# revvu/online_convex_optimization

Measured on AMD Instinct MI355X. Metric: FTRL timesteps/sec (whole node) at d=64, T=1e4; max |regret-ref| error, higher is better.
Workload: dtype f64; 1 GPU; configs[2]: batched FTRL d=64 T=1e4 (1e5-trial job as resident batches of B per GPU); B_per_gpu=32768, T=10000, d=64, coords_per_lane=8, lanes_mode=best, sums=butterfly, comparator=closed form T/2-||theta_T|| (certified per sequence), parallelism=dp1, z_bytes_per_gpu=167772160000

## Files before the change

### include/ocx_testing.h

```cpp
#ifndef OCX_TESTING_H_
#define OCX_TESTING_H_

#include <stdint.h>

#include "ocx.h"

#ifdef __cplusplus
extern "C" {
#endif

int ocx_test_gT_regrets_unclean(uint64_t base_seed, int64_t T, int64_t run0, int64_t R,
                                int64_t d, double eta0, double* regrets, int lanes_per_seq,
                                int device, int64_t unclean_every);

int ocx_test_alg_pipe_chunked(const ocx_layout* L, const double* z_tiled, const double* y_tiled,
                              double eta0, int64_t chunk_steps, double* regret, int* bad,
                              void* stream);

int ocx_test_alg_range(const ocx_layout* L, const double* z_tiled, const double* y_tiled,
                       double eta0, int onepass, int64_t g0, int64_t gn, double* regret,
                       double* gmax, void* stream);

int ocx_test_simulate_alg_etas(const ocx_layout* L, const double* z_tiled, const double* y_tiled,
                               const double* etas, int64_t M, double* regret, double* cum_loss,
                               double* comp_loss, int32_t* closed_out, int flags, int group,
                               void* stream);

int ocx_test_simulate_smart_thresholds(const ocx_layout* L, const double* z_tiled,
                                       const double* y_tiled, const double* thresh, int64_t M,
                                       double eta0, double* regret, int64_t* switch_step,
                                       int flags, unsigned long long* stats, int group,
                                       void* stream);

int64_t ocx_test_trailing_batches(void);

#ifdef __cplusplus
}
#endif
#endif
```

### online_convex_optimization_amd/_lib.py

```python
from __future__ import annotations

import ctypes
import os
import threading

_HERE = os.path.dirname(os.path.abspath(__file__))
LIB_PATH = os.environ.get("OCX_LIB", os.path.join(_HERE, "libocx.so"))

c_dp = ctypes.POINTER(ctypes.c_double)
c_i64p = ctypes.POINTER(ctypes.c_int64)
c_i64 = ctypes.c_int64
c_u64 = ctypes.c_uint64
c_int = ctypes.c_int
c_double = ctypes.c_double
c_vp = ctypes.c_void_p
c_fp = ctypes.POINTER(ctypes.c_float)


class OCXError(RuntimeError):
    """A libocx call failed (bad argument, HIP error, unsupported shape)."""


class Layout(ctypes.Structure):
    _fields_ = [("B", c_i64), ("T", c_i64), ("d", c_i64), ("P", ctypes.c_int32),
# ... 16 lines not shown
    "ocx_simulate_smart_batch": (c_int, [c_dp, c_dp, c_i64, c_i64, c_i64, c_dp, c_double, c_dp,
                                         c_i64p, c_int, c_int]),
    "ocx_ftl_exact_batch": (c_int, [c_dp, c_dp, c_i64, c_i64, c_i64, c_int, c_dp, c_dp, c_dp,
                                    ctypes.POINTER(ctypes.c_int32), c_int, c_int]),
    "ocx_dev_ftl_exact": (c_int, [ctypes.POINTER(Layout), c_vp, c_vp, c_int, c_vp, c_vp, c_vp, c_vp,
                                  c_vp]),
    "ocx_ftl_prefix_actions_batch": (c_int, [c_dp, c_dp, c_i64, c_i64, c_i64, c_int, c_dp,
                                             ctypes.POINTER(ctypes.c_int32), c_int, c_int]),
    "ocx_dev_ftl_prefix_actions": (c_int, [ctypes.POINTER(Layout), c_vp, c_vp, c_int, c_vp, c_vp,
                                           c_vp]),
    "ocx_ftrl_vs_exact_batch": (c_int, [c_dp, c_dp, c_i64, c_i64, c_i64, c_double, c_dp, c_dp,
                                        c_dp, c_dp, c_dp, ctypes.POINTER(ctypes.c_int32), c_int,
                                        c_int]),
    "ocx_ftrl_vs_exact_batch_ex": (c_int, [c_dp, c_dp, c_i64, c_i64, c_i64, c_double, c_dp, c_dp,
                                           c_dp, c_dp, c_dp, ctypes.POINTER(ctypes.c_int32),
                                           c_int, c_int, c_int]),
    "ocx_dev_ftrl_vs_exact": (c_int, [ctypes.POINTER(Layout), c_vp, c_vp, c_double, c_vp, c_vp,
                                      c_vp, c_vp, c_vp, c_vp, c_vp]),
    "ocx_replay_batch": (c_int, [c_dp, c_dp, c_dp, c_i64, c_i64, c_i64, c_dp, c_dp, c_int]),
    "ocx_gT_regrets": (c_int, [c_u64, c_i64, c_i64, c_i64, c_i64, c_double, c_dp, c_int, c_int]),
    "ocx_gT_regrets_dev": (c_int, [c_u64, c_i64, c_i64, c_i64, c_i64, c_double, c_vp, c_int,
                                   c_int]),
    "ocx_gT_max": (c_int, [c_u64, c_i64, c_i64, c_i64, c_i64, c_double, c_int, c_int, c_dp]),
    "ocx_dev_pack": (c_int, [ctypes.POINTER(Layout), c_vp, c_vp, c_vp, c_vp, c_vp]),
    "ocx_dev_gen_gT": (c_int, [ctypes.POINTER(Layout), c_u64, c_i64, c_vp, c_vp, c_vp]),
    "ocx_dev_gen_family": (c_int, [ctypes.POINTER(Layout), c_int, c_vp, c_vp, c_double, c_i64,
                                   c_vp, c_vp, c_vp]),
    "ocx_dev_simulate_alg": (c_int, [ctypes.POINTER(Layout), c_vp, c_vp, c_int, c_double, c_vp,
                                     c_vp, c_vp, c_vp, c_vp, c_vp]),
    "ocx_dev_simulate_smart": (c_int, [ctypes.POINTER(Layout), c_vp, c_vp, c_vp, c_double, c_vp,
                                       c_vp, c_vp]),
    "ocx_dev_simulate_smart_ex": (c_int, [ctypes.POINTER(Layout), c_vp, c_vp, c_vp, c_double,
                                          c_vp, c_vp, c_int, c_vp, c_vp]),
    "ocx_dev_replay": (c_int, [ctypes.POINTER(Layout), ctypes.POINTER(Layout), c_vp, c_vp, c_vp,
                               c_vp, c_vp, c_vp]),
    "ocx_dev_max_regret": (c_int, [c_vp, c_i64, c_vp, c_vp]),
    "ocx_dev_gen_simulate": (c_int, [ctypes.POINTER(Layout), c_u64, c_i64, c_i64, c_vp, c_vp,
                                     c_double, c_vp, c_vp, ctypes.c_uint32, c_i64, c_vp]),
    "ocx_dev_simulate_alg_ex": (c_int, [ctypes.POINTER(Layout), c_vp, c_vp, c_int, c_double, c_vp,
                                        c_vp, c_vp, c_vp, c_vp, c_int, c_vp, c_vp]),
    "ocx_curve_workspace_bytes": (c_i64, [ctypes.POINTER(Layout), c_i64]),
    "ocx_dev_simulate_alg_curve": (c_int, [ctypes.POINTER(Layout), c_vp, c_vp, c_int, c_double,
                                           c_vp, c_i64, c_vp, c_vp, c_vp, c_vp, c_int, c_vp,
                                           ctypes.c_size_t, c_vp]),
    "ocx_simulate_alg_curve_batch": (c_int, [c_dp, c_dp, c_i64, c_i64, c_i64, c_int, c_double,
                                             c_i64p, c_i64, c_dp, c_dp, c_dp,
                                             ctypes.POINTER(ctypes.c_int32), c_int, c_int]),
    "ocx_etas_group": (c_int, [ctypes.POINTER(Layout), c_i64]),
    "ocx_dev_simulate_alg_etas": (c_int, [ctypes.POINTER(Layout), c_vp, c_vp, c_dp, c_i64, c_vp,
                                          c_vp, c_vp, c_vp, c_int, c_vp]),
    "ocx_simulate_alg_etas_batch": (c_int, [c_dp, c_dp, c_i64, c_i64, c_i64, c_dp, c_i64, c_dp,
                                            c_dp, c_dp, ctypes.POINTER(ctypes.c_int32), c_int,
                                            c_int]),
    "ocx_smart_thresholds_group": (c_int, [ctypes.POINTER(Layout), c_i64]),
    "ocx_dev_simulate_smart_thresholds": (c_int, [ctypes.POINTER(Layout), c_vp, c_vp, c_vp, c_i64,
                                                  c_double, c_vp, c_vp, c_int, c_vp, c_vp]),
    "ocx_simulate_smart_thresholds_batch": (c_int, [c_dp, c_dp, c_i64, c_i64, c_i64, c_dp, c_i64,
                                                    c_double, c_dp, c_i64p, c_int, c_int]),
    "ocx_dev_ftrl_vs_exact_ex": (c_int,[ctypes.POINTER(Layout), c_vp, c_vp, c_double, c_vp, c_vp,
                                         c_vp, c_vp, c_vp, c_vp, c_int, c_int, c_vp]),
    "ocx_gT_sweep": (c_int, [c_i64p, c_int, c_i64, c_u64, c_i64, c_double, c_int, c_dp, c_dp]),
    "ocx_gT_sweep_devices": (c_int, [c_i64p, c_int, c_i64, c_u64, c_i64, c_double,
                                     ctypes.POINTER(c_int), c_int, c_int, c_dp, c_dp]),
    "ocx_comparator_loss_blas_batch": (c_int, [c_dp, c_dp, c_dp, c_i64, c_i64, c_i64, c_dp, c_int]),
    "ocx_twin32_batch": (c_int, [c_fp, c_fp, c_i64, c_i64, c_i64, c_int, c_double, c_dp, c_fp,
                                 c_dp, c_fp, c_i64p, c_int]),
    "ocx_dev_twin32": (c_int, [ctypes.POINTER(Layout), c_vp, c_vp, c_int, c_double, c_vp, c_vp,
                               c_vp, c_vp, c_vp, c_vp]),
    "ocx_twin32_gT_regrets": (c_int, [c_u64, c_i64, c_i64, c_i64, c_i64, c_double, c_fp, c_int]),
    "ocx_exact_ball_solve": (c_int, [c_dp, c_dp, c_i64, c_i64, c_i64, c_int, c_int, c_dp, c_dp,
                                     c_dp, c_dp, ctypes.POINTER(ctypes.c_int32), c_int]),
    "ocx_dev_exact_ball_solve": (c_int, [c_vp, c_vp, c_i64, c_i64, c_i64, c_int, c_int, c_vp, c_vp,
                                         c_vp, c_vp, c_vp, c_vp]),
    "ocx_dev_exact_ball_solve_tiled": (c_int, [ctypes.POINTER(Layout), c_vp, c_vp, c_int, c_int,
                                               c_vp, c_vp, c_vp, c_vp, c_vp, c_vp]),
}
TEST_SIGNATURES = {
    "ocx_test_gT_regrets_unclean": (c_int, [c_u64, c_i64, c_i64, c_i64, c_i64, c_double, c_dp,
                                            c_int, c_int, c_i64]),
    "ocx_test_alg_pipe_chunked": (c_int, [ctypes.POINTER(Layout), c_vp, c_vp, c_double, c_i64,
                                          c_vp, c_vp, c_vp]),
    "ocx_test_alg_range": (c_int, [ctypes.POINTER(Layout), c_vp, c_vp, c_double, c_int, c_i64,
                                   c_i64, c_vp, c_vp, c_vp]),
    "ocx_test_simulate_alg_etas": (c_int, [ctypes.POINTER(Layout), c_vp, c_vp, c_dp, c_i64, c_vp,
                                           c_vp, c_vp, c_vp, c_int, c_int, c_vp]),
    "ocx_test_simulate_smart_thresholds": (c_int, [ctypes.POINTER(Layout), c_vp, c_vp, c_vp, c_i64,
                                                   c_double, c_vp, c_vp, c_int, c_vp, c_int,
                                                   c_vp]),
    "ocx_test_trailing_batches": (c_i64, []),
}
OCX_VERSION = 400
OCX_ALG_CLIPPED_ROWS = 1
OCX_EXACT_BALL_MAX_D = 256
OCX_ALG_CLOSED_COMPARATOR = 2
OCX_ALG_TREE_SUMS = 4
OCX_SMART_CLOSED_PREFIX = 8
OCX_GENSIM_SEQUENTIAL = 1
OCX_GENSIM_TWO_PASS = 2

_lib = None
_lock = threading.Lock()


def _share_torch_hip_runtime() -> None:
    if os.environ.get("OCX_NO_TORCH"):
        return
    try:
        import torch
    except ImportError:
        pass


def load():
    global _lib
    if _lib is not None:
        return _lib
    with _lock:
        if _lib is None:
            _share_torch_hip_runtime()
            if not os.path.exists(LIB_PATH):
                raise OCXError(f"libocx.so not found at {LIB_PATH}: the HIP extension is not "
                               "built (python -m online_convex_optimization_amd._build)")
            lib = ctypes.CDLL(LIB_PATH)
            for name, (res, args) in {**SIGNATURES, **TEST_SIGNATURES}.items():
                fn = getattr(lib, name)
                fn.restype = res
                fn.argtypes = args
            if lib.ocx_version() != OCX_VERSION:
                raise OCXError(f"{LIB_PATH} implements ABI version {lib.ocx_version()}, this "
                               f"binding expects {OCX_VERSION}: rebuild the library")
            _lib = lib
    return _lib


def last_error() -> str:
    buf = ctypes.create_string_buffer(4096)
    load().ocx_last_error(buf, len(buf))
    return buf.value.decode(errors="replace")


def check(rc: int, what: str = "") -> None:
    if rc != 0:
        kind = {-1: "invalid argument", -2: "HIP error", -3: "unsupported"}.get(rc, str(rc))
        msg = f"{what}: {kind}: {last_error()}"
        if rc == -1:
            raise ValueError(msg)
        raise OCXError(msg)


def call(name: str, *args) -> None:
    check(getattr(load(), name)(*args), name)


def device_count() -> int:
    n = c_int(0)
    call("ocx_device_count", ctypes.byref(n))
    return int(n.value)


def release_buffers(device: int = 0) -> None:
    call("ocx_release_buffers", int(device))


def layout(B: int, T: int, d: int, lanes_per_seq: int = 0) -> Layout:
    L = Layout()
    call("ocx_layout_init", int(B), int(T), int(d), int(lanes_per_seq), ctypes.byref(L))
# ... 8 lines not shown
```

### online_convex_optimization_amd/csrc/ocx_alg_pipe.h

```cpp
#pragma once
#include <cstdlib>
#include <type_traits>
#include <utility>

#include "ocx_alg_step.h"
#include "ocx_sim_kernels.h"

#ifndef OCX_PIPE_IT32_MAXC
#define OCX_PIPE_IT32_MAXC 4
#endif
template <int C>
using pipe_step_t = typename std::conditional<(C <= OCX_PIPE_IT32_MAXC), int, int64_t>::type;

constexpr int pipe_state_words(int C) { return 2 * C + 7; }

__device__ __forceinline__ int64_t ocx_pipe_wave_id(int64_t gn) {
    const int64_t W = blockDim.x >> 6, blk = blockIdx.x, w = threadIdx.x >> 6;
    const int64_t idle = (int64_t)gridDim.x * W - gn;
    const int64_t full = (int64_t)gridDim.x - idle;
    if (idle <= 0 || full < 0 || blk < full) return blk * W + w;
    return w < W - 1 ? full * W + (blk - full) * (W - 1) + w : gn;
}

struct PipeArgs {
    const double* zt;
    const double* yt;
    int64_t B, T, G;
    double eta0;
    double* regret;
    double* cum_out;
    double* comp_out;
    int* closed_out;
    int onepass;
    int64_t g0, gn;
    int64_t t0, tn;
    double* state;
    int* bad;
    unsigned long long* gmax;
};

#ifndef OCX_PIPE_WAVE_CLOCK
#define OCX_PIPE_WAVE_CLOCK 0
#endif

struct PipeNoObserver {};

template <int C, int P, int NB, bool FTL, bool RT, bool CHUNK = false, class Obs = PipeNoObserver>
__device__ __forceinline__ void alg_pipe_body(const PipeArgs& a, Obs&& obs = Obs{}) {
    static_assert(P >= 2 && NB >= 4, "butterfly layouts, a ring holding z_{t-1} .. z_{t+1}");
    constexpr bool OBS = !std::is_same<typename std::decay<Obs>::type, PipeNoObserver>::value;
    using IT = pipe_step_t<C>;
    constexpr int S = 64 / P;
    constexpr int K = C / 2;
    constexpr int NS = pipe_state_words(C);
    const int lane = threadIdx.x & 63;
    const int64_t wv = (int64_t)__builtin_amdgcn_readfirstlane((int)ocx_pipe_wave_id(a.gn));
    if (wv >= a.gn) return;
    const int64_t g = a.g0 + wv;
    const int64_t T = a.T, t0 = CHUNK ? a.t0 : 0, tn = CHUNK ? a.tn : T;
    const bool first = !CHUNK || t0 == 0, last = !CHUNK || t0 + tn >= T;
    const double eta0 = a.eta0;
#if OCX_PIPE_WAVE_CLOCK
    const uint64_t clk0 = __builtin_amdgcn_s_memrealtime();
#endif
    const int s = lane / P;
    const int c = lane % P;
    const int64_t b = g * S + s;
    const bool live = b < a.B;
    const int64_t tstride = 64;
    const ocx_d2* __restrict__ zg = reinterpret_cast<const ocx_d2*>(a.zt) + (g * T + t0) * tstride;
    const int64_t kst = a.G * T * 64;
    const double* __restrict__ yg = a.yt + (g * T + t0) * S;
    auto stw = [&](int i) -> double& { return a.state[(g * NS + i) * 64 + lane]; };

    double th[C];
    double gp = 0.0;
    double A = 0.0, Bz = 0.0, U = 0.0, V = 0.0, W = 0.0;
    double cum = 0.0;
    bool clean = true;
    ocx_d2 zb[NB][K];
    double yb[NB];
    if (first) {
#pragma unroll
        for (int j = 0; j < C; ++j) th[j] = 0.0;
#pragma unroll
        for (int k = 0; k < K; ++k) zb[NB - 1][k] = ocx_d2{0.0, 0.0};
    } else if constexpr (CHUNK) {
#pragma unroll
        for (int j = 0; j < C; ++j) th[j] = stw(j);
#pragma unroll
        for (int k = 0; k < K; ++k) zb[NB - 1][k] = ocx_d2{stw(C + 2 * k), stw(C + 2 * k + 1)};
        A = stw(2 * C);
        Bz = stw(2 * C + 1);
        V = stw(2 * C + 2);
        W = stw(2 * C + 3);
        gp = stw(2 * C + 4);
        cum = stw(2 * C + 5);
        clean = stw(2 * C + 6) != 0.0;
    }
    auto load = [&](int slot, int64_t tl) {
        const ocx_d2* __restrict__ row = zg + tl * tstride;
#pragma unroll
        for (int k = 0; k < K; ++k) {
#if OCX_LOAD_NT
            zb[slot][k] = __builtin_nontemporal_load(row + k * kst + lane);
#else
            zb[slot][k] = row[k * kst + lane];
#endif
        }
        yb[slot] = yg[tl * S + s];
    };

    double scv = 0.0;

    ocx_ring_loop<NB, true, IT>(tn, load, [&](int u, int64_t tl) {
        const int64_t t = t0 + tl;
        if ((tl & 63) == 0) ocx_pipe_refresh<FTL>(t, lane, eta0, scv, th, U);
        const double zth = __builtin_fma(gp, Bz, A);
        double tth = __builtin_fma(gp, __builtin_fma(gp, W, 2.0 * V), U);
        const ocx_d2* zp1 = zb[(u + NB - 1) % NB];
#pragma unroll
        for (int j = 0; j < C; ++j) th[j] = __builtin_fma(gp, ocx_zj(zp1, j), th[j]);
        if constexpr (OBS) obs.step(t, g, b, c, lane, live, th, cum, clean);
        const double q_raw = ocx_seq_sum<P>(zth);
        double n_raw = ocx_seq_sum<P>(tth);
        double qt;
        if constexpr (!FTL)
            qt = ocx_pipe_q_ftrl<RT>(ocx_readlane(scv, (int)(tl & 63)), q_raw, n_raw);
        else
            qt = ocx_pipe_q_ftl<C, P>(th, q_raw, n_raw, tth, live);
        const double yv = yb[u];
        const double gq = ocx_loss_grad(qt, yv, cum);
        ocx_cert_grad(clean, yv, gq);
        ocx_pipe_advance<P>(th, zb[u], zb[(u + 1) % NB], a.onepass, zth, tth, gq, A, Bz, U, V, W, gp,
                            clean);
    }, CHUNK ? T - t0 : T);
    ocx_d2 zl[K];
    if (tn > 0) ocx_load_tile<C>(zl, zg + (tn - 1) * tstride + lane, kst);
    if constexpr (CHUNK) if (!last) {
#pragma unroll
        for (int j = 0; j < C; ++j) stw(j) = th[j];
#pragma unroll
        for (int k = 0; k < K; ++k) {
            stw(C + 2 * k) = zl[k].x;
            stw(C + 2 * k + 1) = zl[k].y;
        }
        stw(2 * C) = A;
        stw(2 * C + 1) = Bz;
        stw(2 * C + 2) = V;
        stw(2 * C + 3) = W;
        stw(2 * C + 4) = gp;
        stw(2 * C + 5) = cum;
        stw(2 * C + 6) = clean ? 1.0 : 0.0;
        return;
    }
    if (tn > 0) {
#pragma unroll
        for (int j = 0; j < C; ++j) th[j] = __builtin_fma(gp, ocx_zj(zl, j), th[j]);
    }
    if constexpr (OBS) {
        obs.finish(g, b, c, lane, live, th, cum, clean);
        return;
    }

    const bool closed = a.onepass && (clean || !live);
    double comp = 0.0;
    if (__ballot(!closed) != 0) {
        if (first) {
            double xs[C];
            ocx_action_ftl<C, P, false>(th, xs, lane);
            ocx_ring_loop<NB, false, IT>(T, load, [&](int u, int64_t) {
                double p[C];
#pragma unroll
                for (int j = 0; j < C; ++j) p[j] = ocx_zj(zb[u], j) * xs[j];
                const double qq = ocx_total<C, P, false>(p, lane);
                comp += 0.5 * fabs(qq - yb[u]);
            });
        } else if constexpr (CHUNK) {
            comp = __builtin_nan("");
            if (!closed && c == 0 && a.bad) *a.bad = 1;
        }
    }
    if (__ballot(closed) != 0) {
        double p[C];
#pragma unroll
        for (int j = 0; j < C; ++j) p[j] = th[j] * th[j];
        const double nrm = sqrt(ocx_total<C, P, false>(p, lane));
        if (closed) comp = 0.5 * (double)T - nrm;
    }
    if (a.gmax && __ballot(live) != 0) {
        const double rg = cum - comp;
        double mv = (c == 0 && live && rg > 0.0) ? rg : 0.0;
#pragma unroll
        for (int o = 32; o > 0; o >>= 1) {
            const double u = __shfl_xor(mv, o, 64);
            if (u > mv) mv = u;
        }
        if (lane == 0 && mv > 0.0) atomicMax(a.gmax, (unsigned long long)__double_as_longlong(mv));
    }
    if (c == 0 && live) {
        if (a.regret) a.regret[b] = cum - comp;
#if OCX_PIPE_WAVE_CLOCK
        const uint64_t clk1 = __builtin_amdgcn_s_memrealtime();
        if (a.cum_out) a.cum_out[b] = (double)(clk1 - clk0);
        if (a.comp_out) a.comp_out[b] = (double)clk0;
        if (a.closed_out)
            a.closed_out[b] = (int)((__builtin_amdgcn_s_getreg((31 << 11) | 4) & 0xffffu) |
                                    ((__builtin_amdgcn_s_getreg((31 << 11) | 20) & 0xfu) << 16));
#else
        if (a.cum_out) a.cum_out[b] = cum;
        if (a.comp_out) a.comp_out[b] = comp;
        if (a.closed_out) a.closed_out[b] = closed ? 1 : 0;
#endif
    }
}

constexpr bool pipe_layout(int C, int P) {
    return ((P == 8 || P == 16 || P == 32) && (C == 4 || C == 8 || C == 16 || C == 32)) ||
           (P == 64 && C == 16);
}

inline bool ocx_alg_use_pipe(const ocx_layout* L) {
    static const bool no_pipe = [] {
        const char* e = std::getenv("OCX_ALG_NO_PIPE");
        return e && std::atoi(e) != 0;
    }();
    return !no_pipe && ocx_pipe_supported(L);
}

inline int pipe_block_waves(int64_t G) {
    if (std::getenv("OCX_BLOCK_WAVES")) return ocx_block_waves(G);
    return G >= 4 ? 4 : 1;
}

template <int C>
constexpr int pipe_nb(int P) {
    return nb_for(C, P) + 1 < 4 ? 4 : nb_for(C, P) + 1;
}

template <int C, int P, int MINW>
constexpr bool pipe_rt() {
    return !(C == 8 && P == 8 && MINW == 1);
}

template <int C, int P, class F>
bool pipe_dispatch_cp(const ocx_layout* L, F& f, hipError_t& e) {
    if constexpr (pipe_layout(C, P)) {
        if (L->C == C && L->P == P) {
            e = f(std::integral_constant<int, C>{}, std::integral_constant<int, P>{});
            return true;
        }
    }
    return false;
}
template <int C, class F>
bool pipe_dispatch_c(const ocx_layout* L, F& f, hipError_t& e) {
    return pipe_dispatch_cp<C, 8>(L, f, e) || pipe_dispatch_cp<C, 16>(L, f, e) ||
           pipe_dispatch_cp<C, 32>(L, f, e) || pipe_dispatch_cp<C, 64>(L, f, e);
}
template <class F>
hipError_t ocx_pipe_dispatch(const ocx_layout* L, F&& f) {
    hipError_t e = hipErrorInvalidValue;
    (void)(pipe_dispatch_c<4>(L, f, e) || pipe_dispatch_c<8>(L, f, e) ||
           pipe_dispatch_c<16>(L, f, e) || pipe_dispatch_c<32>(L, f, e));
    return e;
}
```

### online_convex_optimization_amd/csrc/ocx_alg_pipe.hip

```cpp
#include <cmath>

#include "ocx_alg_pipe.h"
#include "ocx_device_math.h"
#include "ocx_internal.h"
#include "ocx_sim_kernels.h"

template <int C, int P, int NB, bool FTL, int MINW = 1, bool CHUNK = false>
__global__ __launch_bounds__(OCX_BLOCK, MINW) void ocx_alg_pipe_kernel(PipeArgs a) {
    alg_pipe_body<C, P, NB, FTL, pipe_rt<C, P, MINW>(), CHUNK>(a);
}

namespace {
template <int C, int P>
hipError_t launch_pipe_cp(const PipeArgs& a, int ftl, hipStream_t st) {
    constexpr int NB = pipe_nb<C>(P);
    const int bw = pipe_block_waves(a.gn);
    const dim3 grid = ocx_grid(a.gn, bw), block(64 * bw);
    if (a.state)
        hipLaunchKernelGGL((ocx_alg_pipe_kernel<C, P, NB, false, 1, true>), grid, block, 0, st, a);
    else if (ftl)
        hipLaunchKernelGGL((ocx_alg_pipe_kernel<C, P, NB, true>), grid, block, 0, st, a);
    else
        hipLaunchKernelGGL((ocx_alg_pipe_kernel<C, P, NB, false>), grid, block, 0, st, a);
    return hipGetLastError();
}

hipError_t launch_pipe(const ocx_layout* L, const PipeArgs& a, int ftl, hipStream_t st) {
    if (a.gn <= 0) return hipSuccess;
    return ocx_pipe_dispatch(L, [&](auto c, auto p) {
        return launch_pipe_cp<decltype(c)::value, decltype(p)::value>(a, ftl, st);
    });
}

PipeArgs pipe_args(const ocx_layout* L, const double* zt, const double* yt, double eta0,
                   double* reg, double* cum, double* comp, int* closed_out, int onepass) {
    PipeArgs a{};
    a.zt = zt;
    a.yt = yt;
    a.B = L->B;
    a.T = L->T;
    a.G = L->G;
    a.eta0 = eta0;
    a.regret = reg;
    a.cum_out = cum;
    a.comp_out = comp;
    a.closed_out = closed_out;
    a.onepass = onepass;
    a.g0 = 0;
    a.gn = L->G;
    a.t0 = 0;
    a.tn = L->T;
    return a;
}
}

bool ocx_pipe_supported(const ocx_layout* L) {
    return !L->chain && L->T < ((int64_t)1 << 30) && pipe_layout(L->C, L->P);
}

hipError_t ocx_launch_alg_pipe(const ocx_layout* L, const double* zt, const double* yt, int ftl,
                               double eta0, double* reg, double* cum, double* comp,
                               int* closed_out, int onepass, hipStream_t st) {
    if (L->G == 0) return hipSuccess;
    return launch_pipe(L, pipe_args(L, zt, yt, eta0, reg, cum, comp, closed_out, onepass), ftl, st);
}

int64_t ocx_pipe_state_doubles(const ocx_layout* L) {
    return L->G * 64 * (int64_t)pipe_state_words(L->C);
}

#ifndef OCX_PIPE_LEAN_NB8
#define OCX_PIPE_LEAN_NB8 4
#endif
#ifndef OCX_PIPE_LEAN_NB4
#define OCX_PIPE_LEAN_NB4 8
#endif
bool ocx_pipe_lean_supported(const ocx_layout* L) {
    return !L->chain && L->T < ((int64_t)1 << 30) && ((L->P == 8 && L->C == 8) || (L->P == 16 && L->C == 4));
}

bool ocx_pipe_lean_launchable(const ocx_layout* L) {
    return ocx_pipe_lean_supported(L) || (!L->chain && L->T < ((int64_t)1 << 30) && L->P == 8 && L->C == 4);
}

namespace {
hipError_t launch_lean(const ocx_layout* L, const PipeArgs& a, hipStream_t st) {
    const dim3 grid = ocx_grid(a.gn, 1), block(64);
    if (L->P == 8 && L->C == 4 && !a.state) {
        hipLaunchKernelGGL((ocx_alg_pipe_kernel<4, 8, OCX_PIPE_LEAN_NB4, false, 4>), grid, block, 0, st, a);
    } else if (L->P == 8 && L->C == 8) {
        if (a.state)
            hipLaunchKernelGGL((ocx_alg_pipe_kernel<8, 8, OCX_PIPE_LEAN_NB8, false, 4, true>), grid, block, 0, st, a);
        else
            hipLaunchKernelGGL((ocx_alg_pipe_kernel<8, 8, OCX_PIPE_LEAN_NB8, false, 4>), grid, block, 0, st, a);
    } else if (L->P == 16 && L->C == 4) {
        if (a.state)
            hipLaunchKernelGGL((ocx_alg_pipe_kernel<4, 16, OCX_PIPE_LEAN_NB4, false, 4, true>), grid, block, 0, st, a);
        else
            hipLaunchKernelGGL((ocx_alg_pipe_kernel<4, 16, OCX_PIPE_LEAN_NB4, false, 4>), grid, block, 0, st, a);
    } else {
        return hipErrorInvalidValue;
    }
    return hipGetLastError();
}
}

hipError_t ocx_launch_alg_pipe_lean(const ocx_layout* L, const double* zt, const double* yt,
                                    double eta0, double* reg, int onepass, int64_t g0,
                                    int64_t gn, unsigned long long* gmax, hipStream_t st) {
    if (gn <= 0) return hipSuccess;
    if (g0 < 0 || g0 + gn > L->G) return hipErrorInvalidValue;
    PipeArgs a = pipe_args(L, zt, yt, eta0, reg, nullptr, nullptr, nullptr, onepass);
    a.g0 = g0;
    a.gn = gn;
    a.gmax = gmax;
    return launch_lean(L, a, st);
}

hipError_t ocx_launch_alg_pipe_chunk(const ocx_layout* L, const double* zt, const double* yt,
                                     double eta0, double* reg, int onepass, int64_t t0,
                                     int64_t tn, double* state, int* bad,
                                     unsigned long long* gmax, hipStream_t st) {
    if (L->G == 0 || tn <= 0) return hipSuccess;
    if (t0 < 0 || t0 % 64 != 0 || t0 + tn > L->T || !state || !onepass || !ocx_pipe_supported(L))
        return hipErrorInvalidValue;
    PipeArgs a = pipe_args(L, zt, yt, eta0, reg, nullptr, nullptr, nullptr, onepass);
    a.t0 = t0;
    a.tn = tn;
    a.state = state;
    a.bad = bad;
    a.gmax = t0 + tn >= L->T ? gmax : nullptr;
    return ocx_pipe_lean_supported(L) ? launch_lean(L, a, st) : launch_pipe(L, a, 0, st);
}
```

### online_convex_optimization_amd/csrc/ocx_capi.hip

```cpp
#include <hip/hip_runtime.h>

#include <algorithm>
#include <cstdio>
#include <cstdlib>
#include <cstring>
#include <mutex>
#include <string>
#include <thread>
#include <vector>

#include "../../include/ocx.h"
#include "../../include/ocx_testing.h"
#include "ocx_sim_kernels.h"


namespace {

thread_local std::string g_err;

int fail(int code, const std::string& msg) {
    g_err = msg;
    return code;
}

// ... 1319 lines not shown
                                                pass == 0 ? lin + Bc * 6 : nullptr,
                                                cx->zt.as<double>(), cx->yt.as<double>(), st));
                OCX_HIP(ocx_launch_alg_chunk(&L, cx->zt.as<double>(), cx->yt.as<double>(), t0, 0,
                                             eta0, pass, th, cum, comp,
                                             (pass == 1 && c == nch - 1) ? reg : nullptr, st,
                                             unclean));
            }
        }
        if (dmax) {
            OCX_HIP(launch_max_fold(reg, nb, dmax, st));
        } else if (regrets_on_device) {
            OCX_HIP(hipMemcpyAsync(regrets + r0, reg, (size_t)nb * 8, hipMemcpyDeviceToDevice, st));
        } else {
            OCX_HIP(hipMemcpyAsync(regrets + r0, reg, (size_t)nb * 8, hipMemcpyDeviceToHost, st));
            OCX_HIP(hipStreamSynchronize(st));
        }
    }
    return finish();
}

}

extern "C" {

int ocx_gT_regrets(uint64_t base_seed, int64_t T, int64_t run0, int64_t R, int64_t d,
                   double eta0, double* regrets, int lanes_per_seq, int device) {
    if (!regrets && R > 0) return fail(OCX_E_INVALID, "NULL regrets");
    return gT_run(base_seed, T, run0, R, d, eta0, regrets, nullptr, lanes_per_seq, device);
}

int ocx_gT_regrets_dev(uint64_t base_seed, int64_t T, int64_t run0, int64_t R, int64_t d,
                       double eta0, double* regrets_dev, int lanes_per_seq, int device) {
    if (!regrets_dev && R > 0) return fail(OCX_E_INVALID, "NULL regrets");
    return gT_run(base_seed, T, run0, R, d, eta0, regrets_dev, nullptr, lanes_per_seq, device, 0,
                  true);
}

int ocx_test_alg_pipe_chunked(const ocx_layout* L, const double* z_tiled, const double* y_tiled,
                              double eta0, int64_t chunk_steps, double* regret, int* bad,
                              void* stream) {
    StreamDevice sd_(stream);
    if (int rc = check_layout(L)) return rc;
    if (!ocx_pipe_supported(L)) return fail(OCX_E_UNSUPPORTED, "not a pipelined butterfly layout");
    if (chunk_steps <= 0 || chunk_steps % 64) return fail(OCX_E_INVALID, "chunk_steps: a multiple of 64");
    if (L->B > 0 && (!regret || !bad || !z_tiled || !y_tiled)) return fail(OCX_E_INVALID, "NULL buffer");
    const hipStream_t st = (hipStream_t)stream;
    double* state = nullptr;
    OCX_HIP(hipMalloc(&state, (size_t)std::max<int64_t>(ocx_pipe_state_doubles(L), 1) * 8));
    hipError_t e = hipSuccess;
    for (int64_t t0 = 0; t0 < L->T && e == hipSuccess; t0 += chunk_steps)
        e = ocx_launch_alg_pipe_chunk(L, z_tiled, y_tiled, eta0, regret, 1, t0,
                                      std::min(chunk_steps, L->T - t0), state, bad, nullptr, st);
    const hipError_t es = hipStreamSynchronize(st);
    (void)hipFree(state);
    OCX_HIP(e);
    OCX_HIP(es);
    return OCX_OK;
}

int ocx_test_alg_range(const ocx_layout* L, const double* z_tiled, const double* y_tiled,
                       double eta0, int onepass, int64_t g0, int64_t gn, double* regret,
                       double* gmax, void* stream) {
    StreamDevice sd_(stream);
    if (int rc = check_layout(L)) return rc;
    const bool pipe = ocx_pipe_supported(L);
    if (pipe ? !ocx_pipe_lean_launchable(L) : !(!L->chain && L->P == 8 && L->C == 2))
        return fail(OCX_E_UNSUPPORTED, "not a layout of the pipelines' FTRL range forms");
    if (onepass != 0 && onepass != 1) return fail(OCX_E_INVALID, "onepass must be 0 or 1");
    if (g0 < 0 || gn < 0 || g0 + gn > L->G) return fail(OCX_E_INVALID, "group range outside the layout");
    if (gn > 0 && (!regret || (L->z_elems && (!z_tiled || !y_tiled))))
        return fail(OCX_E_INVALID, "NULL buffer");
    const hipStream_t st = (hipStream_t)stream;
    unsigned long long* gm = reinterpret_cast<unsigned long long*>(gmax);
    const hipError_t e = pipe ? ocx_launch_alg_pipe_lean(L, z_tiled, y_tiled, eta0, regret, onepass,
                                                         g0, gn, gm, st)
                              : ocx_launch_alg_range(L, z_tiled, y_tiled, eta0, regret, onepass, g0,
                                                     gn, gm, st);
    const hipError_t es = hipStreamSynchronize(st);
    OCX_HIP(e);
    OCX_HIP(es);
    return OCX_OK;
}

int64_t ocx_test_trailing_batches(void) { return ocx_trailing_batches_run(); }

int ocx_test_gT_regrets_unclean(uint64_t base_seed, int64_t T, int64_t run0, int64_t R,
                                int64_t d, double eta0, double* regrets, int lanes_per_seq,
                                int device, int64_t unclean_every) {
    if (!regrets && R > 0) return fail(OCX_E_INVALID, "NULL regrets");
    if (unclean_every < 1) return fail(OCX_E_INVALID, "unclean_every must be >= 1");
    return gT_run(base_seed, T, run0, R, d, eta0, regrets, nullptr, lanes_per_seq, device,
                  unclean_every);
}

int ocx_gT_max(uint64_t base_seed, int64_t T, int64_t run0, int64_t R, int64_t d, double eta0,
               int lanes_per_seq, int device, double* gmax) {
    if (!gmax) return fail(OCX_E_INVALID, "NULL gmax");
    return gT_run(base_seed, T, run0, R, d, eta0, nullptr, gmax, lanes_per_seq, device);
}

int ocx_gT_sweep_devices(const int64_t* T_grid, int nT, int64_t runs, uint64_t base_seed,
                         int64_t d, double eta0, const int* devices, int ndev, int lanes_per_seq,
                         double* gmax, double* regrets) {
    if (nT < 0 || runs < 0 || d < 0) return fail(OCX_E_INVALID, "negative argument");
    if (nT == 0) return OCX_OK;
    if (!T_grid || !gmax || !devices || ndev < 1) return fail(OCX_E_INVALID, "NULL argument");
    for (int i = 0; i < nT; ++i)
        if (T_grid[i] < 0) return fail(OCX_E_INVALID, "negative T");
    for (int i = 0; i < nT; ++i) {
        double* row = regrets ? regrets + (size_t)i * runs : nullptr;
        std::vector<double> smax(ndev, 0.0);
        std::vector<int> rc(ndev, OCX_OK);
        std::vector<std::string> err(ndev);
        auto work = [&](int k) {
            const int64_t lo = runs * k / ndev, hi = runs * (k + 1) / ndev;
            rc[k] = gT_run(base_seed, T_grid[i], lo, hi - lo, d, eta0, row ? row + lo : nullptr,
                           row ? nullptr : &smax[k], lanes_per_seq, devices[k]);
            if (rc[k]) err[k] = g_err;
        };
        std::vector<std::thread> th;
        for (int k = 1; k < ndev; ++k) th.emplace_back(work, k);
        work(0);
        for (auto& t : th) t.join();
        for (int k = 0; k < ndev; ++k)
            if (rc[k]) return fail(rc[k], "device " + std::to_string(devices[k]) + ": " + err[k]);
        double m = 0.0;
        if (row) {
            for (int64_t r = 0; r < runs; ++r)
                if (row[r] > m) m = row[r];
        } else {
            for (int k = 0; k < ndev; ++k)
                if (smax[k] > m) m = smax[k];
        }
        gmax[i] = m;
    }
    return OCX_OK;
}

int ocx_gT_sweep(const int64_t* T_grid, int nT, int64_t runs, uint64_t base_seed, int64_t d,
                 double eta0, int ngpus, double* gmax, double* regrets) {
    int n = 0;
    OCX_HIP(hipGetDeviceCount(&n));
    if (ngpus <= 0) ngpus = n;
    if (ngpus > n) return fail(OCX_E_INVALID, "ngpus " + std::to_string(ngpus) +
                                                  " > device count " + std::to_string(n));
    std::vector<int> devs(ngpus);
    for (int k = 0; k < ngpus; ++k) devs[k] = k;
    return ocx_gT_sweep_devices(T_grid, nT, runs, base_seed, d, eta0, devs.data(), ngpus,
                                OCX_LANES_BEST, gmax, regrets);
}

int ocx_comparator_loss_blas_batch(const double* z, const double* y, const double* x, int64_t B,
                                   int64_t T, int64_t d, double* comp_loss, int device) {
    if (B < 0 || T < 0 || d < 0) return fail(OCX_E_INVALID, "negative size");
    if (B == 0) return OCX_OK;
    if ((T * d > 0 && !z) || (T > 0 && !y) || (d > 0 && !x) || !comp_loss)
        return fail(OCX_E_INVALID, "NULL argument");
    DevCtx* cx;
    if (int rc = ctx_enter(device, &cx)) return rc;
    std::lock_guard<std::mutex> lk(cx->mu);
    hipStream_t st = cx->stream;
    const size_t nz = (size_t)(B * T * d), ny = (size_t)(B * T), nx = (size_t)(B * d);
    OCX_HIP(cx->zraw.ensure(nz * 8));
    OCX_HIP(cx->yraw.ensure(ny * 8));
    OCX_HIP(cx->cmp.ensure(nx * 8 + 8));
    OCX_HIP(cx->at.ensure(ny * 8 + 8));
// ... 108 lines not shown
```

### online_convex_optimization_amd/csrc/ocx_sim_kernels.h

```cpp
#pragma once
#include <hip/hip_runtime.h>
#include <stdint.h>

#include "../../include/ocx.h"

bool ocx_supported_C(int C);
hipError_t ocx_launch_alg(const ocx_layout* L, const double* zt, const double* yt, int algo,
                          double eta0, const double* cmp, double* reg, double* cum, double* comp,
                          double* xl, hipStream_t st, double* cmp_out = nullptr,
                          int* regime = nullptr, int onepass = 0, int norm = 0);
bool ocx_pipe_supported(const ocx_layout* L);
hipError_t ocx_launch_alg_pipe(const ocx_layout* L, const double* zt, const double* yt, int ftl,
                               double eta0, double* reg, double* cum, double* comp,
                               int* closed_out, int onepass, hipStream_t st);
int64_t ocx_curve_ws_bytes(const ocx_layout* L, int64_t K);
hipError_t ocx_launch_alg_curve(const ocx_layout* L, const double* zt, const double* yt, int ftl,
                                double eta0, const int64_t* ck, int64_t K, double* reg,
                                double* cum, double* comp, int* closed_out, int onepass,
                                void* ws, hipStream_t st);
bool ocx_etas_instance(const ocx_layout* L, int group);
int ocx_etas_best_group(const ocx_layout* L);
hipError_t ocx_launch_alg_etas(const ocx_layout* L, const double* zt, const double* yt,
                               const double* etas, int64_t M, double* reg, double* cum,
                               double* comp, int* closed_out, int onepass, int group,
                               hipStream_t st);
bool ocx_pipe_lean_supported(const ocx_layout* L);
hipError_t ocx_launch_alg_pipe_lean(const ocx_layout* L, const double* zt, const double* yt,
                                    double eta0, double* reg, int onepass, int64_t g0,
                                    int64_t gn, unsigned long long* gmax, hipStream_t st);
int64_t ocx_pipe_state_doubles(const ocx_layout* L);
hipError_t ocx_launch_alg_pipe_chunk(const ocx_layout* L, const double* zt, const double* yt,
                                     double eta0, double* reg, int onepass, int64_t t0,
                                     int64_t tn, double* state, int* bad,
                                     unsigned long long* gmax, hipStream_t st);
hipError_t ocx_launch_gen_gT_range(const ocx_layout* L, uint64_t base_seed, int64_t run0,
                                   int64_t b_off, int64_t nseq, int wps, double* zt, double* ytl,
                                   hipStream_t st);
bool ocx_pipeline_supported(const ocx_layout* L);
bool ocx_pipeline_worth(const ocx_layout* L, int wps);
bool ocx_stream_fork_ok(hipStream_t st);
hipError_t ocx_launch_gen_gT_range_lr(const ocx_layout* L, uint64_t base_seed, int64_t run0,
                                      int64_t b_off, int64_t nseq, double* zt, double* ytl,
                                      hipStream_t st);
hipError_t ocx_run_gen_rounds(const ocx_layout* L, uint64_t base_seed, int64_t run0, double* zt,
                              double* yt, hipStream_t st);
hipError_t ocx_run_gen_sim_pipelined(const ocx_layout* L, uint64_t base_seed, int64_t run0,
                                     int64_t nbatch, double* zt, double* yt, double eta0,
                                     double* regret, int onepass, unsigned long long* gmax,
                                     int wps, int64_t sub_seqs, hipStream_t st);
bool ocx_pipe_lean_launchable(const ocx_layout* L);
bool ocx_trailing_supported(const ocx_layout* L);
int64_t ocx_trailing_max_batch(const ocx_layout* L);
int64_t ocx_trailing_batches_run();
hipError_t ocx_run_gen_sim_trailing(const ocx_layout* L, uint64_t base_seed, int64_t run0,
                                    int64_t nbatch, double* zt, double* yt0, double* yt1,
                                    uint64_t* gst, double* fst, int* bad, double eta0,
                                    double* regret, int64_t last_B, unsigned long long* gmax,
                                    int nchunks, hipStream_t st);
hipError_t ocx_launch_gen_gT_rows(const ocx_layout* L, uint64_t base_seed, int64_t run0,
                                  int64_t t_off, int64_t nrows, const uint64_t* st_in,
                                  uint64_t* st_out, int labels, double* zt, double* ytl,
                                  hipStream_t st);
hipError_t ocx_launch_exact_wide(const double* z, const double* y, int64_t B, int64_t T,
                                 int64_t d, int tiled, int P, int C, int S, int64_t G, int norm,
                                 int all_prefixes, double* actions, double* obj, double* gap,
                                 double* step_loss, int32_t* info, hipStream_t st);
hipError_t ocx_launch_exact_polish(const double* z, const double* y, int64_t B, int64_t T,
                                   int64_t d, int tiled, int P, int C, int S, int64_t G, int norm,
                                   int all_prefixes, double* actions, double* obj, double* gap,
                                   double* step_loss, hipStream_t st);
hipError_t ocx_launch_exact_big(const double* z, const double* y, int64_t B, int64_t T, int64_t d,
                                int tiled, int P, int C, int S, int64_t G, int norm,
                                int all_prefixes, double* actions, double* obj, double* gap,
                                double* step_loss, int32_t* info, hipStream_t st);
hipError_t ocx_launch_smart(const ocx_layout* L, const double* zt, const double* yt,
                            const double* th, double eta0, double* reg, int64_t* sw,
                            hipStream_t st);
hipError_t ocx_launch_smart_closed(const ocx_layout* L, const double* zt, const double* yt,
                                   const double* th, double eta0, double* reg, int64_t* sw,
                                   int closed_prefix, int closed_comp, unsigned long long* stats,
                                   hipStream_t st);
bool ocx_thresholds_instance(const ocx_layout* L, int group);
int ocx_thresholds_best_group(const ocx_layout* L);
hipError_t ocx_launch_smart_thresholds(const ocx_layout* L, const double* zt, const double* yt,
                                       const double* th, int64_t M, double eta0, double* reg,
                                       int64_t* sw, int closed_prefix, int closed_comp,
                                       unsigned long long* stats, int group, hipStream_t st);
hipError_t ocx_launch_smart_wave(const ocx_layout* L, const double* zt, const double* yt,
                                 const double* th, double eta0, double* reg, int64_t* sw,
                                 hipStream_t st);
hipError_t ocx_launch_replay(const ocx_layout* L, const double* zt, const double* yt,
                             const double* at, double* cum, double* comp, hipStream_t st);
hipError_t ocx_launch_prefix_actions(const ocx_layout* L, const double* zt, const double* yt,
                                     double* actions, int* regime, hipStream_t st, int norm = 0);
hipError_t ocx_launch_pack(const ocx_layout* L, const double* z, const double* y, double* zt,
                           double* ytl, hipStream_t st);
hipError_t ocx_launch_max(const double* r, int64_t B, double* out, hipStream_t st);
// ... 40 lines not shown
```

Measured before the change: 12.70 billion timesteps/s.

## Add persistent grid-stride pipelined FTRL kernel with LDS-capped occupancy for C=8,P=8

Adds a persistent variant of the pipelined FTRL kernel. A fixed grid of waves loops over groups with a grid stride, replacing one wave per group when the group count exceeds one full occupancy round. Residency is capped per CU by reserving dynamic LDS, and the kernel uses a smaller ring (NB=4) and a different launch-bounds minimum. The goal is fewer resident waves per CU, which allows more registers per wave, and to avoid the tail imbalance of the last round. The cost is lower latency hiding and extra host-side occupancy queries, which are cached per device.

```diff
diff --git a/include/ocx_testing.h b/include/ocx_testing.h
--- a/include/ocx_testing.h
+++ b/include/ocx_testing.h
@@ -21,6 +21,10 @@
                        double eta0, int onepass, int64_t g0, int64_t gn, double* regret,
                        double* gmax, void* stream);
 
+int ocx_test_alg_pipe_persistent(const ocx_layout* L, const double* z_tiled, const double* y_tiled,
+                                 int ftl, double eta0, int onepass, int64_t nwaves, double* regret,
+                                 double* cum, double* comp, int32_t* closed_out, void* stream);
+
 int ocx_test_simulate_alg_etas(const ocx_layout* L, const double* z_tiled, const double* y_tiled,
                                const double* etas, int64_t M, double* regret, double* cum_loss,
                                double* comp_loss, int32_t* closed_out, int flags, int group,
diff --git a/online_convex_optimization_amd/_lib.py b/online_convex_optimization_amd/_lib.py
--- a/online_convex_optimization_amd/_lib.py
+++ b/online_convex_optimization_amd/_lib.py
@@ -122,6 +122,8 @@
                                           c_vp, c_vp, c_vp]),
     "ocx_test_alg_range": (c_int, [ctypes.POINTER(Layout), c_vp, c_vp, c_double, c_int, c_i64,
                                    c_i64, c_vp, c_vp, c_vp]),
+    "ocx_test_alg_pipe_persistent": (c_int, [ctypes.POINTER(Layout), c_vp, c_vp, c_int, c_double,
+                                             c_int, c_i64, c_vp, c_vp, c_vp, c_vp, c_vp]),
     "ocx_test_simulate_alg_etas": (c_int, [ctypes.POINTER(Layout), c_vp, c_vp, c_dp, c_i64, c_vp,
                                            c_vp, c_vp, c_vp, c_int, c_int, c_vp]),
     "ocx_test_simulate_smart_thresholds": (c_int, [ctypes.POINTER(Layout), c_vp, c_vp, c_vp, c_i64,
diff --git a/online_convex_optimization_amd/csrc/ocx_alg_pipe.h b/online_convex_optimization_amd/csrc/ocx_alg_pipe.h
--- a/online_convex_optimization_amd/csrc/ocx_alg_pipe.h
+++ b/online_convex_optimization_amd/csrc/ocx_alg_pipe.h
@@ -33,6 +33,7 @@
     int* closed_out;
     int onepass;
     int64_t g0, gn;
+    int64_t gstride;
     int64_t t0, tn;
     double* state;
     int* bad;
@@ -45,8 +46,8 @@
 
 struct PipeNoObserver {};
 
-template <int C, int P, int NB, bool FTL, bool RT, bool CHUNK = false, class Obs = PipeNoObserver>
-__device__ __forceinline__ void alg_pipe_body(const PipeArgs& a, Obs&& obs = Obs{}) {
+template <int C, int P, int NB, bool FTL, bool RT, bool CHUNK, class Obs>
+__device__ __forceinline__ void alg_pipe_group(const PipeArgs& a, const int64_t wv, Obs& obs) {
     static_assert(P >= 2 && NB >= 4, "butterfly layouts, a ring holding z_{t-1} .. z_{t+1}");
     constexpr bool OBS = !std::is_same<typename std::decay<Obs>::type, PipeNoObserver>::value;
     using IT = pipe_step_t<C>;
@@ -54,8 +55,6 @@
     constexpr int K = C / 2;
     constexpr int NS = pipe_state_words(C);
     const int lane = threadIdx.x & 63;
-    const int64_t wv = (int64_t)__builtin_amdgcn_readfirstlane((int)ocx_pipe_wave_id(a.gn));
-    if (wv >= a.gn) return;
     const int64_t g = a.g0 + wv;
     const int64_t T = a.T, t0 = CHUNK ? a.t0 : 0, tn = CHUNK ? a.tn : T;
     const bool first = !CHUNK || t0 == 0, last = !CHUNK || t0 + tn >= T;
@@ -215,6 +214,22 @@
     }
 }
 
+template <int C, int P, int NB, bool FTL, bool RT, bool CHUNK = false, class Obs = PipeNoObserver,
+          bool LOOP = false>
+__device__ __forceinline__ void alg_pipe_body(const PipeArgs& a, Obs&& obs = Obs{}) {
+    if constexpr (!LOOP) {
+        const int64_t wv = (int64_t)__builtin_amdgcn_readfirstlane((int)ocx_pipe_wave_id(a.gn));
+        if (wv >= a.gn) return;
+        alg_pipe_group<C, P, NB, FTL, RT, CHUNK>(a, wv, obs);
+    } else {
+        static_assert(!CHUNK, "a chunked run carries one group's state per wave");
+        const int64_t w0 = (int64_t)__builtin_amdgcn_readfirstlane((int)ocx_wave_id());
+        if (w0 >= a.gstride) return;
+        for (int64_t wv = w0; wv < a.gn; wv += a.gstride)
+            alg_pipe_group<C, P, NB, FTL, RT, CHUNK>(a, wv, obs);
+    }
+}
+
 constexpr bool pipe_layout(int C, int P) {
     return ((P == 8 || P == 16 || P == 32) && (C == 4 || C == 8 || C == 16 || C == 32)) ||
            (P == 64 && C == 16);
diff --git a/online_convex_optimization_amd/csrc/ocx_alg_pipe.hip b/online_convex_optimization_amd/csrc/ocx_alg_pipe.hip
--- a/online_convex_optimization_amd/csrc/ocx_alg_pipe.hip
+++ b/online_convex_optimization_amd/csrc/ocx_alg_pipe.hip
@@ -1,19 +1,127 @@
 #include <cmath>
+#include <map>
+#include <mutex>
 
 #include "ocx_alg_pipe.h"
 #include "ocx_device_math.h"
 #include "ocx_internal.h"
 #include "ocx_sim_kernels.h"
 
-template <int C, int P, int NB, bool FTL, int MINW = 1, bool CHUNK = false>
+template <int C, int P, int NB, bool FTL, int MINW = 1, bool CHUNK = false, bool LOOP = false>
 __global__ __launch_bounds__(OCX_BLOCK, MINW) void ocx_alg_pipe_kernel(PipeArgs a) {
-    alg_pipe_body<C, P, NB, FTL, pipe_rt<C, P, MINW>(), CHUNK>(a);
+    alg_pipe_body<C, P, NB, FTL, pipe_rt<C, P, MINW>(), CHUNK, PipeNoObserver, LOOP>(a);
+}
+
+#ifndef OCX_PIPE_PERS_NB
+#define OCX_PIPE_PERS_NB 4
+#endif
+#ifndef OCX_PIPE_PERS_MINW
+#define OCX_PIPE_PERS_MINW 2
+#endif
+#ifndef OCX_PIPE_PERS_WPS
+#define OCX_PIPE_PERS_WPS 1
+#endif
+#ifndef OCX_PIPE_PERS_TUNE
+#define OCX_PIPE_PERS_TUNE 0
+#endif
+
+template <int C, int P>
+constexpr bool pipe_persistent_layout() {
+    return C == 8 && P == 8;
 }
 
 namespace {
+struct PersGeom {
+    hipError_t err = hipSuccess;
+    int64_t round = 0;
+    int64_t nw = 0;
+    size_t lds = 0;
+};
+
+template <class K>
+hipError_t pers_shape(K kern, int dev, int cus, int wps, int bw, PersGeom& gm) {
+    const int want = wps * 4 / bw;
+    int lds_cu = 0, q = 0;
+    if (hipDeviceGetAttribute(&lds_cu, hipDeviceAttributeMaxSharedMemoryPerMultiprocessor, dev) !=
+            hipSuccess || lds_cu <= 0)
+        lds_cu = 160 * 1024;
+    hipError_t e = hipOccupancyMaxActiveBlocksPerMultiprocessor(&q, kern, 64 * bw, 0);
+    if (e != hipSuccess) return e;
+    size_t lds = 0;
+    if (q > want) {
+        for (lds = ((size_t)lds_cu / (want + 1) / 512 + 1) * 512; lds <= (size_t)lds_cu; lds += 512) {
+            e = hipOccupancyMaxActiveBlocksPerMultiprocessor(&q, kern, 64 * bw, lds);
+            if (e != hipSuccess) return e;
+            if (q <= want) break;
+        }
+    }
+    if (q <= 0 || q > want) return hipErrorInvalidConfiguration;
+    gm.lds = lds;
+    gm.nw = (int64_t)q * bw * cus;
+    return hipSuccess;
+}
+
+template <int C, int P>
+PersGeom pers_geometry(int ftl) {
+    constexpr int NB = pipe_nb<C>(P), NBP = OCX_PIPE_PERS_NB, MW = OCX_PIPE_PERS_MINW;
+    PersGeom gm;
+    int dev = 0, cus = 0;
+    if ((gm.err = hipGetDevice(&dev)) != hipSuccess) return gm;
+    int wps = OCX_PIPE_PERS_WPS, bw = 4;
+#if OCX_PIPE_PERS_TUNE
+    if (const char* e = std::getenv("OCX_PIPE_PERS_WPS")) wps = std::atoi(e);
+    if (const char* e = std::getenv("OCX_PIPE_PERS_BW")) bw = std::atoi(e);
+    if (wps < 1 || wps > 8 || (bw != 1 && bw != 4)) return gm.err = hipErrorInvalidValue, gm;
+#else
+    static std::mutex mu;
+    static std::map<std::pair<int, int>, PersGeom> cache;
+    std::lock_guard<std::mutex> lk(mu);
+    const auto key = std::make_pair(dev, ftl);
+    const auto it = cache.find(key);
+    if (it != cache.end()) return it->second;
+#endif
+    if ((gm.err = hipDeviceGetAttribute(&cus, hipDeviceAttributeMultiprocessorCount, dev)) != hipSuccess)
+        return gm;
+    int q = 0;
+    gm.err = ftl ? hipOccupancyMaxActiveBlocksPerMultiprocessor(&q, ocx_alg_pipe_kernel<C, P, NB, true>, 256, 0)
+                 : hipOccupancyMaxActiveBlocksPerMultiprocessor(&q, ocx_alg_pipe_kernel<C, P, NB, false>, 256, 0);
+    if (gm.err != hipSuccess) return gm;
+    gm.round = (int64_t)q * 4 * cus;
+    gm.err = ftl ? pers_shape(ocx_alg_pipe_kernel<C, P, NBP, true, MW, false, true>, dev, cus, wps, bw, gm)
+                 : pers_shape(ocx_alg_pipe_kernel<C, P, NBP, false, MW, false, true>, dev, cus, wps, bw, gm);
+#if !OCX_PIPE_PERS_TUNE
+    if (gm.err == hipSuccess) cache.emplace(key, gm);
+#endif
+    return gm;
+}
+
+template <int C, int P>
+hipError_t launch_pipe_persistent(PipeArgs a, int ftl, int64_t nwaves, const PersGeom& gm,
+                                  hipStream_t st) {
+    constexpr int NBP = OCX_PIPE_PERS_NB, MW = OCX_PIPE_PERS_MINW;
+    int bw = 4;
+#if OCX_PIPE_PERS_TUNE
+    if (const char* e = std::getenv("OCX_PIPE_PERS_BW")) bw = std::atoi(e) == 1 ? 1 : 4;
+#endif
+    a.gstride = nwaves > 0 ? nwaves : gm.nw;
+    const dim3 grid = ocx_grid(a.gstride, bw), block(64 * bw);
+    if (ftl)
+        hipLaunchKernelGGL((ocx_alg_pipe_kernel<C, P, NBP, true, MW, false, true>), grid, block, gm.lds, st, a);
+    else
+        hipLaunchKernelGGL((ocx_alg_pipe_kernel<C, P, NBP, false, MW, false, true>), grid, block, gm.lds, st, a);
+    return hipGetLastError();
+}
+
 template <int C, int P>
 hipError_t launch_pipe_cp(const PipeArgs& a, int ftl, hipStream_t st) {
     constexpr int NB = pipe_nb<C>(P);
+    if constexpr (pipe_persistent_layout<C, P>()) {
+        if (!a.state) {
+            const PersGeom gm = pers_geometry<C, P>(ftl);
+            if (gm.err != hipSuccess) return gm.err;
+            if (a.gn > gm.round) return launch_pipe_persistent<C, P>(a, ftl, 0, gm, st);
+        }
+    }
     const int bw = pipe_block_waves(a.gn);
     const dim3 grid = ocx_grid(a.gn, bw), block(64 * bw);
     if (a.state)
@@ -48,6 +156,7 @@
     a.onepass = onepass;
     a.g0 = 0;
     a.gn = L->G;
+    a.gstride = L->G;
     a.t0 = 0;
     a.tn = L->T;
     return a;
@@ -63,6 +172,22 @@
                                int* closed_out, int onepass, hipStream_t st) {
     if (L->G == 0) return hipSuccess;
     return launch_pipe(L, pipe_args(L, zt, yt, eta0, reg, cum, comp, closed_out, onepass), ftl, st);
+}
+
+bool ocx_pipe_persistent_supported(const ocx_layout* L) {
+    return ocx_pipe_supported(L) && L->C == 8 && L->P == 8;
+}
+
+hipError_t ocx_launch_alg_pipe_persistent(const ocx_layout* L, const double* zt, const double* yt,
+                                          int ftl, double eta0, double* reg, double* cum,
+                                          double* comp, int* closed_out, int onepass,
+                                          int64_t nwaves, hipStream_t st) {
+    if (!ocx_pipe_persistent_supported(L) || nwaves <= 0) return hipErrorInvalidValue;
+    if (L->G == 0) return hipSuccess;
+    const PersGeom gm = pers_geometry<8, 8>(ftl);
+    if (gm.err != hipSuccess) return gm.err;
+    return launch_pipe_persistent<8, 8>(pipe_args(L, zt, yt, eta0, reg, cum, comp, closed_out, onepass),
+                                        ftl, nwaves, gm, st);
 }
 
 int64_t ocx_pipe_state_doubles(const ocx_layout* L) {
diff --git a/online_convex_optimization_amd/csrc/ocx_capi.hip b/online_convex_optimization_amd/csrc/ocx_capi.hip
--- a/online_convex_optimization_amd/csrc/ocx_capi.hip
+++ b/online_convex_optimization_amd/csrc/ocx_capi.hip
@@ -1425,6 +1425,27 @@
     return OCX_OK;
 }
 
+int ocx_test_alg_pipe_persistent(const ocx_layout* L, const double* z_tiled, const double* y_tiled,
+                                 int ftl, double eta0, int onepass, int64_t nwaves, double* regret,
+                                 double* cum, double* comp, int32_t* closed_out, void* stream) {
+    StreamDevice sd_(stream);
+    if (int rc = check_layout(L)) return rc;
+    if (!ocx_pipe_persistent_supported(L))
+        return fail(OCX_E_UNSUPPORTED, "no persistent instance of the pipelined kernel for this layout");
+    if ((ftl != 0 && ftl != 1) || (onepass != 0 && onepass != 1))
+        return fail(OCX_E_INVALID, "ftl and onepass must be 0 or 1");
+    if (nwaves < 1 || nwaves > ((int64_t)1 << 20)) return fail(OCX_E_INVALID, "nwaves: 1 .. 2^20");
+    if (L->B > 0 && (!regret || (L->z_elems && (!z_tiled || !y_tiled))))
+        return fail(OCX_E_INVALID, "NULL buffer");
+    const hipStream_t st = (hipStream_t)stream;
+    const hipError_t e = ocx_launch_alg_pipe_persistent(L, z_tiled, y_tiled, ftl, eta0, regret, cum,
+                                                        comp, closed_out, onepass, nwaves, st);
+    const hipError_t es = hipStreamSynchronize(st);
+    OCX_HIP(e);
+    OCX_HIP(es);
+    return OCX_OK;
+}
+
 int64_t ocx_test_trailing_batches(void) { return ocx_trailing_batches_run(); }
 
 int ocx_test_gT_regrets_unclean(uint64_t base_seed, int64_t T, int64_t run0, int64_t R,
diff --git a/online_convex_optimization_amd/csrc/ocx_sim_kernels.h b/online_convex_optimization_amd/csrc/ocx_sim_kernels.h
--- a/online_convex_optimization_amd/csrc/ocx_sim_kernels.h
+++ b/online_convex_optimization_amd/csrc/ocx_sim_kernels.h
@@ -13,6 +13,11 @@
 hipError_t ocx_launch_alg_pipe(const ocx_layout* L, const double* zt, const double* yt, int ftl,
                                double eta0, double* reg, double* cum, double* comp,
                                int* closed_out, int onepass, hipStream_t st);
+bool ocx_pipe_persistent_supported(const ocx_layout* L);
+hipError_t ocx_launch_alg_pipe_persistent(const ocx_layout* L, const double* zt, const double* yt,
+                                          int ftl, double eta0, double* reg, double* cum,
+                                          double* comp, int* closed_out, int onepass,
+                                          int64_t nwaves, hipStream_t st);
 int64_t ocx_curve_ws_bytes(const ocx_layout* L, int64_t K);
 hipError_t ocx_launch_alg_curve(const ocx_layout* L, const double* zt, const double* yt, int ftl,
                                 double eta0, const int64_t* ck, int64_t K, double* reg,
```

Result: faster. 12.92 billion timesteps/s (median of 6 runs) (+1.7%).
